# Lakonik/SSDNeRF

Hardware: NVIDIA H100
Metric: rays/sec (128^2 render) & DDIM triplanes/sec (higher is better)
Workload: dtype fp16 tensor-core UNet (fp32 accumulate), fp32 renderer

## Files before the change

ssdnerf_b200/csrc/conv_row2.cu:

```cuda
#include "common.cuh"
#include "tc_common.cuh"
#include "conv_row_epilogue.cuh"
#include "../../include/ssdnerf_b200.h"
#include <cuda_fp16.h>

namespace ssdnerf {
using namespace tc;

constexpr int kRwThreads = 384;
constexpr int kRwRowSlot = 17 * 1024;
constexpr int kRwBSlot = kRwN * 128;
constexpr int kRwRows = 6, kRwBStages = 6;
constexpr size_t kRwSmem = (size_t)kRwRows * kRwRowSlot + (size_t)kRwBStages * kRwBSlot + 1024  + 256  +
                           256  + 512 ;

struct ConvRowParams {
    uint32_t B, H;
    const __half* x1; uint32_t C1;
    const __half* x2; uint32_t C2;
    long long xs1[3], xs2[3];
    const float* bias;
    const __half* residual;
    __half* out;
    float* qstats;
};

__global__ void __launch_bounds__(kRwThreads, 1)
k_conv_row2(const __grid_constant__ CUtensorMap mapB, const ConvRowParams p) {
    extern __shared__ uint8_t smem_raw[];
    uint8_t* smem = reinterpret_cast<uint8_t*>(((uintptr_t)smem_raw + 1023) & ~(uintptr_t)1023);
    uint8_t* sR = smem;
    uint8_t* sB = smem + kRwRows * kRwRowSlot;
    uint64_t* fullR = reinterpret_cast<uint64_t*>(sB + kRwBStages * kRwBSlot);
    uint64_t* emptyR = fullR + kRwRows;
    uint64_t* fullB = emptyR + kRwRows;
    uint64_t* emptyB = fullB + kRwBStages;
    float* qacc = reinterpret_cast<float*>(reinterpret_cast<uint8_t*>(fullR) + 256);
    float* sbias = qacc + 64;

    const int warp = threadIdx.x >> 5, lane = threadIdx.x & 31, wg = warp >> 2;
    const uint32_t tiles_per_img = p.H / 2, total_tiles = p.B * tiles_per_img;
    const uint32_t kc1 = p.C1 / 64, KC = (p.C1 + p.C2) / 64;
    const uint32_t tile0 = blockIdx.x, tstep = gridDim.x;
    const uint32_t my_tiles = tile0 < total_tiles ? (total_tiles - tile0 + tstep - 1) / tstep : 0;

    if (threadIdx.x == 0) {
        prefetch_tmap(&mapB);
        for (int i = 0; i < kRwRows; ++i) { mbar_init(&fullR[i], 4); mbar_init(&emptyR[i], 8); }
        for (int i = 0; i < kRwBStages; ++i) { mbar_init(&fullB[i], 1); mbar_init(&emptyB[i], 8); }
        fence_mbar_init();
    }
    for (int i = threadIdx.x; i < 64; i += kRwThreads) qacc[i] = 0.0f;
    for (int i = threadIdx.x; i < kRwN; i += kRwThreads) sbias[i] = p.bias ? __ldg(p.bias + i) : 0.0f;
    __syncthreads();
    pdl_trigger();
    pdl_wait();

    if (wg == 2) {
        setmaxnreg_dec<120>();
        const uint32_t lt = threadIdx.x - 256u;
        const uint32_t c8 = lt & 7u, p0 = lt >> 3;
        uint32_t idx = 0;
        for (uint32_t tile = tile0; tile < total_tiles; tile += tstep) {
            const uint32_t b = tile / tiles_per_img, y0 = (tile - b * tiles_per_img) * 2;
            for (uint32_t j = 0; j < KC; ++j) {
                const bool first = j < kc1;
                const __half* src = first ? p.x1 : p.x2;
                const long long xs0 = first ? p.xs1[0] : p.xs2[0], xs1 = first ? p.xs1[1] : p.xs2[1], xs2 = first ? p.xs1[2] : p.xs2[2];
                const uint32_t cl = (first ? j : j - kc1) * 64u + c8 * 8u;
                for (uint32_t r = 0; r < 4; ++r) {
                    const int y = (int)(y0 + r) - 1;
                    const bool row_ok = y >= 0 && y < (int)p.H;
                    const __half* rowp = src + (long long)b * xs2 + (long long)(row_ok ? y : 0) * xs1 + cl;
                    uint4 v[9];
#pragma unroll
                    for (int n = 0; n < 9; ++n) {
                        const int x = (int)(p0 + 16u * n) - 1;
                        v[n] = (row_ok && (unsigned)x < (unsigned)kRwW) ? __ldg(reinterpret_cast<const uint4*>(rowp + (long long)x * xs0))
                                                                       : make_uint4(0, 0, 0, 0);
                    }
                    const uint32_t slot = idx % kRwRows;
                    mbar_wait(&emptyR[slot], ((idx / kRwRows) & 1u) ^ 1u);
                    const uint32_t dst = smem_u32(sR + slot * kRwRowSlot);
#pragma unroll
                    for (int n = 0; n < 9; ++n) {
                        const uint32_t px = p0 + 16u * n;
                        if (px >= 130u) continue;
                        sts128(dst + px * 128u + ((c8 ^ (px & 7u)) << 4), v[n]);
                    }
                    __syncwarp();
                    if (lane == 0) mbar_arrive(&fullR[slot]);
                    ++idx;
                }
            }
        }
    } else {
        setmaxnreg_inc<192>();
        const uint32_t a = (uint32_t)wg, wq = (uint32_t)warp & 3u, cq = (uint32_t)lane & 3u;
        const uint32_t steps_per_tile = KC * 9u, total_steps = my_tiles * steps_per_tile;
        auto issue_w = [&](uint32_t L) {
            const uint32_t s = L % kRwBStages;
            if (L >= (uint32_t)kRwBStages) mbar_wait(&emptyB[s], ((L / kRwBStages) - 1u) & 1u);
            mbar_expect_tx(&fullB[s], (uint32_t)kRwBSlot);
            const uint32_t rem = L % steps_per_tile;
            tma_load_4d(sB + s * kRwBSlot, &mapB, &fullB[s], (int)((rem / 9u) * 64u), 0, (int)(rem % 9u), 0);
        };
        if (threadIdx.x == 0)
            for (uint32_t L = 0; L < total_steps && L < (uint32_t)kRwBStages; ++L) issue_w(L);
        auto release_row = [&](uint32_t ring) { if (lane == 0) mbar_arrive(&emptyR[ring % kRwRows]); };
        uint32_t m = 0, ridx = 0;
        const uint32_t lrow = wq * 16u + ((uint32_t)lane & 15u);
        const uint32_t lk = (uint32_t)lane >> 4;
        for (uint32_t tile = tile0; tile < total_tiles; tile += tstep) {
            const uint32_t b = tile / tiles_per_img, y0 = (tile - b * tiles_per_img) * 2;
            float acc0[64], acc1[64];
#pragma unroll
            for (int i = 0; i < 64; ++i) { acc0[i] = 0.0f; acc1[i] = 0.0f; }
            for (uint32_t j = 0; j < KC; ++j) {
                const uint32_t unused = ridx + (a == 0 ? 3u : 0u);
                if (a == 1) { mbar_wait(&fullR[unused % kRwRows], (unused / kRwRows) & 1u); release_row(unused); }
                for (uint32_t ky = 0; ky < 3; ++ky) {
                    const uint32_t ring = ridx + ky + a;
                    mbar_wait(&fullR[ring % kRwRows], (ring / kRwRows) & 1u);
                    const uint32_t rowS = smem_u32(sR + (ring % kRwRows) * kRwRowSlot);
                    for (uint32_t kx = 0; kx < 3; ++kx) {
                        const uint32_t sb = m % kRwBStages;
                        uint32_t af[2][4][4];
#pragma unroll
                        for (uint32_t h = 0; h < 2; ++h) {
                            const uint32_t px = 64u * h + lrow + kx;
#pragma unroll
                            for (uint32_t k = 0; k < 4; ++k) ldmatrix_x4(rowS + px * 128u + (((2u * k + lk) ^ (px & 7u)) << 4), af[h][k]);
                        }
                        if (kx == 2) release_row(ring);
                        mbar_wait(&fullB[sb], (m / kRwBStages) & 1u);
                        const uint64_t b_desc = make_desc_sw128(smem_u32(sB + sb * kRwBSlot));
                        wgmma_fence();
                        fence_regs(acc0); fence_regs(acc1);
#pragma unroll
                        for (uint32_t k = 0; k < 4; ++k) {
                            wgmma_rs_n128(acc0, af[0][k], b_desc + 2 * k, 1u);
                            wgmma_rs_n128(acc1, af[1][k], b_desc + 2 * k, 1u);
                        }
                        wgmma_commit();
                        wgmma_wait<0>();
                        fence_regs(acc0); fence_regs(acc1);
                        if (lane == 0) mbar_arrive(&emptyB[sb]);
                        if (threadIdx.x == 0 && m >= 1 && m - 1 + kRwBStages < total_steps) issue_w(m - 1 + kRwBStages);
                        ++m;
                    }
                }
                if (a == 0) { mbar_wait(&fullR[unused % kRwRows], (unused / kRwRows) & 1u); release_row(unused); }
                ridx += 4;
            }
            const size_t pix0 = ((size_t)b * p.H + y0 + a) * kRwW;
#pragma unroll
            for (int i = 0; i < 16; ++i) {
                const uint32_t ch = 8u * i + 2u * cq;
                const float b0 = sbias[ch], b1 = sbias[ch + 1];
                float su = 0.0f, sq = 0.0f;
#pragma unroll
                for (int h = 0; h < 2; ++h) {
#pragma unroll
                    for (int hh = 0; hh < 2; ++hh) {
                        const size_t o = (pix0 + 64u * h + wq * 16u + ((uint32_t)lane >> 2) + 8u * hh) * kRwN + ch;
                        float v0 = (h ? acc1 : acc0)[4 * i + 2 * hh] + b0, v1 = (h ? acc1 : acc0)[4 * i + 2 * hh + 1] + b1;
                        if (p.residual) { const float2 r = __half22float2(*reinterpret_cast<const __half2*>(p.residual + o)); v0 += r.x; v1 += r.y; }
                        *reinterpret_cast<__half2*>(p.out + o) = __floats2half2_rn(v0, v1);
                        su += v0 + v1; sq = fmaf(v0, v0, fmaf(v1, v1, sq));
                    }
                }
                if (p.qstats) {
                    frag_quad_reduce(su, sq);
                    if ((lane & ~2) == 0) { float* qa = qacc + (2 * i + (lane >> 1)) * 2; atomicAdd(qa, su); atomicAdd(qa + 1, sq); }
                }
            }
            if (p.qstats) {
                asm volatile("bar.sync 1, 256;" ::: "memory");
                if (threadIdx.x < 64) {
                    const float val = qacc[threadIdx.x];
                    if (val != 0.0f) atomicAdd(p.qstats + (size_t)b * 64 + threadIdx.x, val);
                    qacc[threadIdx.x] = 0.0f;
                }
                asm volatile("bar.sync 1, 256;" ::: "memory");
            }
        }
    }
    __syncthreads();
}

int make_map_4d_box(CUtensorMap* m, const void* base, uint64_t K, uint64_t e1, uint64_t e2, uint64_t e3, uint64_t s1, uint64_t s2, uint64_t s3,
                    uint32_t x1, uint32_t x2, uint32_t x3);

static int launch_row2(const CUtensorMap& mB, const ConvRowParams& p, int sms, cudaStream_t stream) {
    static DeviceOnce attr;
    if (attr.first()) {
        SSDNERF_CUDA_OK(cudaFuncSetAttribute(k_conv_row2, cudaFuncAttributeMaxDynamicSharedMemorySize, (int)kRwSmem));
    }
    const uint32_t total = p.B * (p.H / 2);
    SSDNERF_CUDA_OK(launch_pdl(k_conv_row2, dim3(total < (uint32_t)sms ? total : (uint32_t)sms), dim3(kRwThreads), kRwSmem, stream, mB, p));
    SSDNERF_LAUNCH_OK();
    return 0;
}

int conv_row2_launch(const ssdnerf_gemm_args* a, int sms, cudaStream_t stream) {
    if (((uintptr_t)a->a1 & 15u) || ((a->a1_strides[0] | a->a1_strides[1] | a->a1_strides[2]) & 15u) ||
        (a->a2 && (((uintptr_t)a->a2 & 15u) || ((a->a2_strides[0] | a->a2_strides[1] | a->a2_strides[2]) & 15u))) ||
        ((uintptr_t)a->out & 3u) || ((uintptr_t)a->residual & 3u))
        return set_error_msg(SSDNERF_ERR_ARG, "gemm: row-pair convolution needs 16-byte aligned inputs and strides, 4-byte aligned output / residual");
    ConvRowParams p{};
    p.B = a->d3; p.H = a->d2;
    p.x1 = (const __half*)a->a1; p.C1 = a->k1;
    p.x2 = (const __half*)a->a2; p.C2 = a->a2 ? a->k2 : 0;
    for (int i = 0; i < 3; ++i) { p.xs1[i] = (long long)(a->a1_strides[i] / 2); p.xs2[i] = a->a2 ? (long long)(a->a2_strides[i] / 2) : 0; }
    p.bias = a->bias_n; p.residual = (const __half*)a->residual; p.out = (__half*)a->out; p.qstats = a->qstats;
    const uint64_t ktot = (uint64_t)a->k1 + (a->a2 ? a->k2 : 0);
    CUtensorMap mB;
    if (int e = make_map_4d_box(&mB, a->b, ktot, a->n_rows_b ? a->n_rows_b : a->n, a->bx2 ? a->bx2 : 1, a->bx3 ? a->bx3 : 1, a->b_strides[0],
                                a->b_strides[1], a->b_strides[2], kRwN, 1, 1)) return e;
    return launch_row2(mB, p, sms, stream);
}

}
```

ssdnerf_b200/csrc/tc_common.cuh:

```cuda
#pragma once
#include <cuda.h>
#include <cuda_runtime.h>
#include <stdint.h>

namespace ssdnerf {
namespace tc {

__device__ __forceinline__ uint32_t smem_u32(const void* p) { return (uint32_t)__cvta_generic_to_shared(p); }

__device__ __forceinline__ void sts128(uint32_t addr, const uint4& v) {
    asm volatile("st.shared.v4.b32 [%0], {%1, %2, %3, %4};" ::"r"(addr), "r"(v.x), "r"(v.y), "r"(v.z), "r"(v.w) : "memory");
}

__device__ __forceinline__ void mbar_init(uint64_t* bar, uint32_t count) {
    asm volatile("mbarrier.init.shared::cta.b64 [%0], %1;" ::"r"(smem_u32(bar)), "r"(count));
}
__device__ __forceinline__ void fence_mbar_init() { asm volatile("fence.mbarrier_init.release.cluster;" ::: "memory"); }
__device__ __forceinline__ void mbar_arrive(uint64_t* bar) {
    asm volatile("mbarrier.arrive.shared::cta.b64 _, [%0];" ::"r"(smem_u32(bar)) : "memory");
}
__device__ __forceinline__ void mbar_wait(uint64_t* bar, uint32_t parity) {
    uint32_t spins = 0, ok = 0;
    while (!ok) {
        asm volatile(
            "{\n\t.reg .pred p;\n\t"
            "mbarrier.try_wait.parity.acquire.cluster.shared::cta.b64 p, [%1], %2;\n\t"
            "selp.b32 %0, 1, 0, p;\n\t}"
            : "=r"(ok) : "r"(smem_u32(bar)), "r"(parity) : "memory");
        if (!ok && ++spins > 200000000u) { asm volatile("trap;"); }
    }
}
__device__ __forceinline__ void mbar_expect_tx(uint64_t* bar, uint32_t bytes) {
    asm volatile("mbarrier.arrive.expect_tx.shared::cta.b64 _, [%0], %1;" ::"r"(smem_u32(bar)), "r"(bytes) : "memory");
}

__device__ __forceinline__ void prefetch_tmap(const CUtensorMap* m) {
    asm volatile("prefetch.tensormap [%0];" ::"l"(reinterpret_cast<uint64_t>(m)) : "memory");
}
__device__ __forceinline__ void tma_load_4d(void* dst, const CUtensorMap* m, uint64_t* bar, int c0, int c1, int c2, int c3) {
    asm volatile(
        "cp.async.bulk.tensor.4d.shared::cluster.global.mbarrier::complete_tx::bytes [%0], [%1, {%3, %4, %5, %6}], [%2];"
        ::"r"(smem_u32(dst)), "l"(reinterpret_cast<uint64_t>(m)), "r"(smem_u32(bar)), "r"(c0), "r"(c1), "r"(c2), "r"(c3)
        : "memory");
}
__device__ __forceinline__ void fence_proxy_async_smem() { asm volatile("fence.proxy.async.shared::cta;" ::: "memory"); }

template <int N> __device__ __forceinline__ void setmaxnreg_inc() { asm volatile("setmaxnreg.inc.sync.aligned.u32 %0;" ::"n"(N)); }
template <int N> __device__ __forceinline__ void setmaxnreg_dec() { asm volatile("setmaxnreg.dec.sync.aligned.u32 %0;" ::"n"(N)); }

__device__ __forceinline__ uint64_t make_desc_sw128(uint32_t smem_addr) {
    uint64_t d = 0;
    d |= (uint64_t)((smem_addr >> 4) & 0x3FFFu);
    d |= (uint64_t)1 << 16;
    d |= (uint64_t)(1024u >> 4) << 32;
    d |= (uint64_t)1 << 62;
    return d;
}
__device__ __forceinline__ void wgmma_fence() { asm volatile("wgmma.fence.sync.aligned;" ::: "memory"); }
__device__ __forceinline__ void wgmma_commit() { asm volatile("wgmma.commit_group.sync.aligned;" ::: "memory"); }
template <int N> __device__ __forceinline__ void wgmma_wait() { asm volatile("wgmma.wait_group.sync.aligned %0;" ::"n"(N) : "memory"); }
template <int R> __device__ __forceinline__ void fence_regs(float (&d)[R]) {
#pragma unroll
    for (int i = 0; i < R; ++i) asm volatile("" : "+f"(d[i])::"memory");
}

__device__ __forceinline__ void ldmatrix_x4(uint32_t addr, uint32_t (&r)[4]) {
    asm volatile("ldmatrix.sync.aligned.m8n8.x4.shared.b16 {%0, %1, %2, %3}, [%4];"
                 : "=r"(r[0]), "=r"(r[1]), "=r"(r[2]), "=r"(r[3]) : "r"(addr) : "memory");
}

__device__ __forceinline__ void wgmma_ss_n64(float (&d)[32], uint64_t a_desc, uint64_t b_desc, uint32_t accumulate) {
    asm volatile(
        "{\n\t.reg .pred p;\n\t"
        "setp.ne.b32 p, %34, 0;\n\t"
        "wgmma.mma_async.sync.aligned.m64n64k16.f32.f16.f16 "
        "{%0, %1, %2, %3, %4, %5, %6, %7, %8, %9, %10, %11, %12, %13, %14, %15, %16, %17, %18, %19, %20, %21, %22, %23, %24, %25, %26, %27, %28, %29, %30, %31}, %32, %33, p, 1, 1, 0, 0;\n\t}"
        : "+f"(d[0]), "+f"(d[1]), "+f"(d[2]), "+f"(d[3]), "+f"(d[4]), "+f"(d[5]), "+f"(d[6]), "+f"(d[7]), "+f"(d[8]), "+f"(d[9]), "+f"(d[10]), "+f"(d[11]), "+f"(d[12]), "+f"(d[13]), "+f"(d[14]), "+f"(d[15]), "+f"(d[16]), "+f"(d[17]), "+f"(d[18]), "+f"(d[19]), "+f"(d[20]), "+f"(d[21]), "+f"(d[22]), "+f"(d[23]), "+f"(d[24]), "+f"(d[25]), "+f"(d[26]), "+f"(d[27]), "+f"(d[28]), "+f"(d[29]), "+f"(d[30]), "+f"(d[31])
        : "l"(a_desc), "l"(b_desc), "r"(accumulate));
}
__device__ __forceinline__ void wgmma_ss_n128(float (&d)[64], uint64_t a_desc, uint64_t b_desc, uint32_t accumulate) {
    asm volatile(
        "{\n\t.reg .pred p;\n\t"
        "setp.ne.b32 p, %66, 0;\n\t"
        "wgmma.mma_async.sync.aligned.m64n128k16.f32.f16.f16 "
        "{%0, %1, %2, %3, %4, %5, %6, %7, %8, %9, %10, %11, %12, %13, %14, %15, %16, %17, %18, %19, %20, %21, %22, %23, %24, %25, %26, %27, %28, %29, %30, %31, %32, %33, %34, %35, %36, %37, %38, %39, %40, %41, %42, %43, %44, %45, %46, %47, %48, %49, %50, %51, %52, %53, %54, %55, %56, %57, %58, %59, %60, %61, %62, %63}, %64, %65, p, 1, 1, 0, 0;\n\t}"
        : "+f"(d[0]), "+f"(d[1]), "+f"(d[2]), "+f"(d[3]), "+f"(d[4]), "+f"(d[5]), "+f"(d[6]), "+f"(d[7]), "+f"(d[8]), "+f"(d[9]), "+f"(d[10]), "+f"(d[11]), "+f"(d[12]), "+f"(d[13]), "+f"(d[14]), "+f"(d[15]), "+f"(d[16]), "+f"(d[17]), "+f"(d[18]), "+f"(d[19]), "+f"(d[20]), "+f"(d[21]), "+f"(d[22]), "+f"(d[23]), "+f"(d[24]), "+f"(d[25]), "+f"(d[26]), "+f"(d[27]), "+f"(d[28]), "+f"(d[29]), "+f"(d[30]), "+f"(d[31]), "+f"(d[32]), "+f"(d[33]), "+f"(d[34]), "+f"(d[35]), "+f"(d[36]), "+f"(d[37]), "+f"(d[38]), "+f"(d[39]), "+f"(d[40]), "+f"(d[41]), "+f"(d[42]), "+f"(d[43]), "+f"(d[44]), "+f"(d[45]), "+f"(d[46]), "+f"(d[47]), "+f"(d[48]), "+f"(d[49]), "+f"(d[50]), "+f"(d[51]), "+f"(d[52]), "+f"(d[53]), "+f"(d[54]), "+f"(d[55]), "+f"(d[56]), "+f"(d[57]), "+f"(d[58]), "+f"(d[59]), "+f"(d[60]), "+f"(d[61]), "+f"(d[62]), "+f"(d[63])
        : "l"(a_desc), "l"(b_desc), "r"(accumulate));
}
__device__ __forceinline__ void wgmma_rs_n128(float (&d)[64], const uint32_t (&a)[4], uint64_t b_desc, uint32_t accumulate) {
    asm volatile(
        "{\n\t.reg .pred p;\n\t"
        "setp.ne.b32 p, %69, 0;\n\t"
        "wgmma.mma_async.sync.aligned.m64n128k16.f32.f16.f16 "
        "{%0, %1, %2, %3, %4, %5, %6, %7, %8, %9, %10, %11, %12, %13, %14, %15, %16, %17, %18, %19, %20, %21, %22, %23, %24, %25, %26, %27, %28, %29, %30, %31, %32, %33, %34, %35, %36, %37, %38, %39, %40, %41, %42, %43, %44, %45, %46, %47, %48, %49, %50, %51, %52, %53, %54, %55, %56, %57, %58, %59, %60, %61, %62, %63}, {%64, %65, %66, %67}, %68, p, 1, 1, 0;\n\t}"
        : "+f"(d[0]), "+f"(d[1]), "+f"(d[2]), "+f"(d[3]), "+f"(d[4]), "+f"(d[5]), "+f"(d[6]), "+f"(d[7]), "+f"(d[8]), "+f"(d[9]), "+f"(d[10]), "+f"(d[11]), "+f"(d[12]), "+f"(d[13]), "+f"(d[14]), "+f"(d[15]), "+f"(d[16]), "+f"(d[17]), "+f"(d[18]), "+f"(d[19]), "+f"(d[20]), "+f"(d[21]), "+f"(d[22]), "+f"(d[23]), "+f"(d[24]), "+f"(d[25]), "+f"(d[26]), "+f"(d[27]), "+f"(d[28]), "+f"(d[29]), "+f"(d[30]), "+f"(d[31]), "+f"(d[32]), "+f"(d[33]), "+f"(d[34]), "+f"(d[35]), "+f"(d[36]), "+f"(d[37]), "+f"(d[38]), "+f"(d[39]), "+f"(d[40]), "+f"(d[41]), "+f"(d[42]), "+f"(d[43]), "+f"(d[44]), "+f"(d[45]), "+f"(d[46]), "+f"(d[47]), "+f"(d[48]), "+f"(d[49]), "+f"(d[50]), "+f"(d[51]), "+f"(d[52]), "+f"(d[53]), "+f"(d[54]), "+f"(d[55]), "+f"(d[56]), "+f"(d[57]), "+f"(d[58]), "+f"(d[59]), "+f"(d[60]), "+f"(d[61]), "+f"(d[62]), "+f"(d[63])
        : "r"(a[0]), "r"(a[1]), "r"(a[2]), "r"(a[3]), "l"(b_desc), "r"(accumulate));
}
__device__ __forceinline__ void wgmma_ss_n256(float (&d)[128], uint64_t a_desc, uint64_t b_desc, uint32_t accumulate) {
    asm volatile(
        "{\n\t.reg .pred p;\n\t"
        "setp.ne.b32 p, %130, 0;\n\t"
        "wgmma.mma_async.sync.aligned.m64n256k16.f32.f16.f16 "
        "{%0, %1, %2, %3, %4, %5, %6, %7, %8, %9, %10, %11, %12, %13, %14, %15, %16, %17, %18, %19, %20, %21, %22, %23, %24, %25, %26, %27, %28, %29, %30, %31, %32, %33, %34, %35, %36, %37, %38, %39, %40, %41, %42, %43, %44, %45, %46, %47, %48, %49, %50, %51, %52, %53, %54, %55, %56, %57, %58, %59, %60, %61, %62, %63, %64, %65, %66, %67, %68, %69, %70, %71, %72, %73, %74, %75, %76, %77, %78, %79, %80, %81, %82, %83, %84, %85, %86, %87, %88, %89, %90, %91, %92, %93, %94, %95, %96, %97, %98, %99, %100, %101, %102, %103, %104, %105, %106, %107, %108, %109, %110, %111, %112, %113, %114, %115, %116, %117, %118, %119, %120, %121, %122, %123, %124, %125, %126, %127}, %128, %129, p, 1, 1, 0, 0;\n\t}"
        : "+f"(d[0]), "+f"(d[1]), "+f"(d[2]), "+f"(d[3]), "+f"(d[4]), "+f"(d[5]), "+f"(d[6]), "+f"(d[7]), "+f"(d[8]), "+f"(d[9]), "+f"(d[10]), "+f"(d[11]), "+f"(d[12]), "+f"(d[13]), "+f"(d[14]), "+f"(d[15]), "+f"(d[16]), "+f"(d[17]), "+f"(d[18]), "+f"(d[19]), "+f"(d[20]), "+f"(d[21]), "+f"(d[22]), "+f"(d[23]), "+f"(d[24]), "+f"(d[25]), "+f"(d[26]), "+f"(d[27]), "+f"(d[28]), "+f"(d[29]), "+f"(d[30]), "+f"(d[31]), "+f"(d[32]), "+f"(d[33]), "+f"(d[34]), "+f"(d[35]), "+f"(d[36]), "+f"(d[37]), "+f"(d[38]), "+f"(d[39]), "+f"(d[40]), "+f"(d[41]), "+f"(d[42]), "+f"(d[43]), "+f"(d[44]), "+f"(d[45]), "+f"(d[46]), "+f"(d[47]), "+f"(d[48]), "+f"(d[49]), "+f"(d[50]), "+f"(d[51]), "+f"(d[52]), "+f"(d[53]), "+f"(d[54]), "+f"(d[55]), "+f"(d[56]), "+f"(d[57]), "+f"(d[58]), "+f"(d[59]), "+f"(d[60]), "+f"(d[61]), "+f"(d[62]), "+f"(d[63]), "+f"(d[64]), "+f"(d[65]), "+f"(d[66]), "+f"(d[67]), "+f"(d[68]), "+f"(d[69]), "+f"(d[70]), "+f"(d[71]), "+f"(d[72]), "+f"(d[73]), "+f"(d[74]), "+f"(d[75]), "+f"(d[76]), "+f"(d[77]), "+f"(d[78]), "+f"(d[79]), "+f"(d[80]), "+f"(d[81]), "+f"(d[82]), "+f"(d[83]), "+f"(d[84]), "+f"(d[85]), "+f"(d[86]), "+f"(d[87]), "+f"(d[88]), "+f"(d[89]), "+f"(d[90]), "+f"(d[91]), "+f"(d[92]), "+f"(d[93]), "+f"(d[94]), "+f"(d[95]), "+f"(d[96]), "+f"(d[97]), "+f"(d[98]), "+f"(d[99]), "+f"(d[100]), "+f"(d[101]), "+f"(d[102]), "+f"(d[103]), "+f"(d[104]), "+f"(d[105]), "+f"(d[106]), "+f"(d[107]), "+f"(d[108]), "+f"(d[109]), "+f"(d[110]), "+f"(d[111]), "+f"(d[112]), "+f"(d[113]), "+f"(d[114]), "+f"(d[115]), "+f"(d[116]), "+f"(d[117]), "+f"(d[118]), "+f"(d[119]), "+f"(d[120]), "+f"(d[121]), "+f"(d[122]), "+f"(d[123]), "+f"(d[124]), "+f"(d[125]), "+f"(d[126]), "+f"(d[127])
        : "l"(a_desc), "l"(b_desc), "r"(accumulate));
}

__device__ __forceinline__ void wgmma_ss_n16(float (&d)[8], uint64_t a_desc, uint64_t b_desc, uint32_t accumulate) {
    asm volatile(
        "{\n\t.reg .pred p;\n\t"
        "setp.ne.b32 p, %10, 0;\n\t"
        "wgmma.mma_async.sync.aligned.m64n16k16.f32.f16.f16 "
        "{%0, %1, %2, %3, %4, %5, %6, %7}, %8, %9, p, 1, 1, 0, 0;\n\t}"
        : "+f"(d[0]), "+f"(d[1]), "+f"(d[2]), "+f"(d[3]), "+f"(d[4]), "+f"(d[5]), "+f"(d[6]), "+f"(d[7])
        : "l"(a_desc), "l"(b_desc), "r"(accumulate));
}
__device__ __forceinline__ void wgmma_ss_n40(float (&d)[20], uint64_t a_desc, uint64_t b_desc, uint32_t accumulate) {
    asm volatile(
        "{\n\t.reg .pred p;\n\t"
        "setp.ne.b32 p, %22, 0;\n\t"
        "wgmma.mma_async.sync.aligned.m64n40k16.f32.f16.f16 "
        "{%0, %1, %2, %3, %4, %5, %6, %7, %8, %9, %10, %11, %12, %13, %14, %15, %16, %17, %18, %19}, %20, %21, p, 1, 1, 0, 0;\n\t}"
        : "+f"(d[0]), "+f"(d[1]), "+f"(d[2]), "+f"(d[3]), "+f"(d[4]), "+f"(d[5]), "+f"(d[6]), "+f"(d[7]), "+f"(d[8]), "+f"(d[9]), "+f"(d[10]), "+f"(d[11]), "+f"(d[12]), "+f"(d[13]), "+f"(d[14]), "+f"(d[15]), "+f"(d[16]), "+f"(d[17]), "+f"(d[18]), "+f"(d[19])
        : "l"(a_desc), "l"(b_desc), "r"(accumulate));
}
__device__ __forceinline__ void wgmma_ss_n48(float (&d)[24], uint64_t a_desc, uint64_t b_desc, uint32_t accumulate) {
    asm volatile(
        "{\n\t.reg .pred p;\n\t"
        "setp.ne.b32 p, %26, 0;\n\t"
        "wgmma.mma_async.sync.aligned.m64n48k16.f32.f16.f16 "
        "{%0, %1, %2, %3, %4, %5, %6, %7, %8, %9, %10, %11, %12, %13, %14, %15, %16, %17, %18, %19, %20, %21, %22, %23}, %24, %25, p, 1, 1, 0, 0;\n\t}"
        : "+f"(d[0]), "+f"(d[1]), "+f"(d[2]), "+f"(d[3]), "+f"(d[4]), "+f"(d[5]), "+f"(d[6]), "+f"(d[7]), "+f"(d[8]), "+f"(d[9]), "+f"(d[10]), "+f"(d[11]), "+f"(d[12]), "+f"(d[13]), "+f"(d[14]), "+f"(d[15]), "+f"(d[16]), "+f"(d[17]), "+f"(d[18]), "+f"(d[19]), "+f"(d[20]), "+f"(d[21]), "+f"(d[22]), "+f"(d[23])
        : "l"(a_desc), "l"(b_desc), "r"(accumulate));
}
__device__ __forceinline__ void wgmma_ss_n80(float (&d)[40], uint64_t a_desc, uint64_t b_desc, uint32_t accumulate) {
    asm volatile(
        "{\n\t.reg .pred p;\n\t"
        "setp.ne.b32 p, %42, 0;\n\t"
        "wgmma.mma_async.sync.aligned.m64n80k16.f32.f16.f16 "
        "{%0, %1, %2, %3, %4, %5, %6, %7, %8, %9, %10, %11, %12, %13, %14, %15, %16, %17, %18, %19, %20, %21, %22, %23, %24, %25, %26, %27, %28, %29, %30, %31, %32, %33, %34, %35, %36, %37, %38, %39}, %40, %41, p, 1, 1, 0, 0;\n\t}"
        : "+f"(d[0]), "+f"(d[1]), "+f"(d[2]), "+f"(d[3]), "+f"(d[4]), "+f"(d[5]), "+f"(d[6]), "+f"(d[7]), "+f"(d[8]), "+f"(d[9]), "+f"(d[10]), "+f"(d[11]), "+f"(d[12]), "+f"(d[13]), "+f"(d[14]), "+f"(d[15]), "+f"(d[16]), "+f"(d[17]), "+f"(d[18]), "+f"(d[19]), "+f"(d[20]), "+f"(d[21]), "+f"(d[22]), "+f"(d[23]), "+f"(d[24]), "+f"(d[25]), "+f"(d[26]), "+f"(d[27]), "+f"(d[28]), "+f"(d[29]), "+f"(d[30]), "+f"(d[31]), "+f"(d[32]), "+f"(d[33]), "+f"(d[34]), "+f"(d[35]), "+f"(d[36]), "+f"(d[37]), "+f"(d[38]), "+f"(d[39])
        : "l"(a_desc), "l"(b_desc), "r"(accumulate));
}
__device__ __forceinline__ void wgmma_ss_n160(float (&d)[80], uint64_t a_desc, uint64_t b_desc, uint32_t accumulate) {
    asm volatile(
        "{\n\t.reg .pred p;\n\t"
        "setp.ne.b32 p, %82, 0;\n\t"
        "wgmma.mma_async.sync.aligned.m64n160k16.f32.f16.f16 "
        "{%0, %1, %2, %3, %4, %5, %6, %7, %8, %9, %10, %11, %12, %13, %14, %15, %16, %17, %18, %19, %20, %21, %22, %23, %24, %25, %26, %27, %28, %29, %30, %31, %32, %33, %34, %35, %36, %37, %38, %39, %40, %41, %42, %43, %44, %45, %46, %47, %48, %49, %50, %51, %52, %53, %54, %55, %56, %57, %58, %59, %60, %61, %62, %63, %64, %65, %66, %67, %68, %69, %70, %71, %72, %73, %74, %75, %76, %77, %78, %79}, %80, %81, p, 1, 1, 0, 0;\n\t}"
        : "+f"(d[0]), "+f"(d[1]), "+f"(d[2]), "+f"(d[3]), "+f"(d[4]), "+f"(d[5]), "+f"(d[6]), "+f"(d[7]), "+f"(d[8]), "+f"(d[9]), "+f"(d[10]), "+f"(d[11]), "+f"(d[12]), "+f"(d[13]), "+f"(d[14]), "+f"(d[15]), "+f"(d[16]), "+f"(d[17]), "+f"(d[18]), "+f"(d[19]), "+f"(d[20]), "+f"(d[21]), "+f"(d[22]), "+f"(d[23]), "+f"(d[24]), "+f"(d[25]), "+f"(d[26]), "+f"(d[27]), "+f"(d[28]), "+f"(d[29]), "+f"(d[30]), "+f"(d[31]), "+f"(d[32]), "+f"(d[33]), "+f"(d[34]), "+f"(d[35]), "+f"(d[36]), "+f"(d[37]), "+f"(d[38]), "+f"(d[39]), "+f"(d[40]), "+f"(d[41]), "+f"(d[42]), "+f"(d[43]), "+f"(d[44]), "+f"(d[45]), "+f"(d[46]), "+f"(d[47]), "+f"(d[48]), "+f"(d[49]), "+f"(d[50]), "+f"(d[51]), "+f"(d[52]), "+f"(d[53]), "+f"(d[54]), "+f"(d[55]), "+f"(d[56]), "+f"(d[57]), "+f"(d[58]), "+f"(d[59]), "+f"(d[60]), "+f"(d[61]), "+f"(d[62]), "+f"(d[63]), "+f"(d[64]), "+f"(d[65]), "+f"(d[66]), "+f"(d[67]), "+f"(d[68]), "+f"(d[69]), "+f"(d[70]), "+f"(d[71]), "+f"(d[72]), "+f"(d[73]), "+f"(d[74]), "+f"(d[75]), "+f"(d[76]), "+f"(d[77]), "+f"(d[78]), "+f"(d[79])
        : "l"(a_desc), "l"(b_desc), "r"(accumulate));
}

}
}
```

Before: 97.87 million.

## Switch row conv to SS wgmma with one-deep async pipelining and batched residual loads

Replaces the ldmatrix-fed register-A wgmma with shared-memory descriptors for A, which removes the per-step ldmatrix traffic and register pressure. It keeps one wgmma group in flight (wait<1>) and defers releasing B stages and rows until the next step, so the tensor cores no longer stall on each step's completion. Because the producer's generic stores are now read by the async proxy, it adds a proxy fence. The epilogue also batches the residual loads ahead of use. In exchange, weight prefetch is issued one stage later, and the 130-pixel row layout must line up with the SW128 descriptor stride.

```diff
diff --git a/ssdnerf_b200/csrc/conv_row2.cu b/ssdnerf_b200/csrc/conv_row2.cu
--- a/ssdnerf_b200/csrc/conv_row2.cu
+++ b/ssdnerf_b200/csrc/conv_row2.cu
@@ -88,6 +88,7 @@
                         if (px >= 130u) continue;
                         sts128(dst + px * 128u + ((c8 ^ (px & 7u)) << 4), v[n]);
                     }
+                    fence_proxy_async_smem();
                     __syncwarp();
                     if (lane == 0) mbar_arrive(&fullR[slot]);
                     ++idx;
@@ -108,9 +109,14 @@
         if (threadIdx.x == 0)
             for (uint32_t L = 0; L < total_steps && L < (uint32_t)kRwBStages; ++L) issue_w(L);
         auto release_row = [&](uint32_t ring) { if (lane == 0) mbar_arrive(&emptyR[ring % kRwRows]); };
+        constexpr uint32_t kNone = 0xFFFFFFFFu;
+        uint32_t pend_b = kNone, pend_row = kNone;
+        auto retire = [&]() {
+            if (pend_b != kNone && lane == 0) mbar_arrive(&emptyB[pend_b]);
+            if (pend_row != kNone) release_row(pend_row);
+            pend_b = kNone; pend_row = kNone;
+        };
         uint32_t m = 0, ridx = 0;
-        const uint32_t lrow = wq * 16u + ((uint32_t)lane & 15u);
-        const uint32_t lk = (uint32_t)lane >> 4;
         for (uint32_t tile = tile0; tile < total_tiles; tile += tstep) {
             const uint32_t b = tile / tiles_per_img, y0 = (tile - b * tiles_per_img) * 2;
             float acc0[64], acc1[64];
@@ -125,54 +131,69 @@
                     const uint32_t rowS = smem_u32(sR + (ring % kRwRows) * kRwRowSlot);
                     for (uint32_t kx = 0; kx < 3; ++kx) {
                         const uint32_t sb = m % kRwBStages;
-                        uint32_t af[2][4][4];
-#pragma unroll
-                        for (uint32_t h = 0; h < 2; ++h) {
-                            const uint32_t px = 64u * h + lrow + kx;
-#pragma unroll
-                            for (uint32_t k = 0; k < 4; ++k) ldmatrix_x4(rowS + px * 128u + (((2u * k + lk) ^ (px & 7u)) << 4), af[h][k]);
-                        }
-                        if (kx == 2) release_row(ring);
+                        const uint64_t a_desc0 = make_desc_sw128(rowS + kx * 128u), a_desc1 = make_desc_sw128(rowS + (64u + kx) * 128u);
                         mbar_wait(&fullB[sb], (m / kRwBStages) & 1u);
                         const uint64_t b_desc = make_desc_sw128(smem_u32(sB + sb * kRwBSlot));
                         wgmma_fence();
                         fence_regs(acc0); fence_regs(acc1);
 #pragma unroll
                         for (uint32_t k = 0; k < 4; ++k) {
-                            wgmma_rs_n128(acc0, af[0][k], b_desc + 2 * k, 1u);
-                            wgmma_rs_n128(acc1, af[1][k], b_desc + 2 * k, 1u);
+                            wgmma_ss_n128(acc0, a_desc0 + 2 * k, b_desc + 2 * k, 1u);
+                            wgmma_ss_n128(acc1, a_desc1 + 2 * k, b_desc + 2 * k, 1u);
                         }
                         wgmma_commit();
-                        wgmma_wait<0>();
                         fence_regs(acc0); fence_regs(acc1);
-                        if (lane == 0) mbar_arrive(&emptyB[sb]);
-                        if (threadIdx.x == 0 && m >= 1 && m - 1 + kRwBStages < total_steps) issue_w(m - 1 + kRwBStages);
+                        wgmma_wait<1>();
+                        retire();
+                        pend_b = sb;
+                        pend_row = kx == 2 ? ring : kNone;
+                        if (threadIdx.x == 0 && m >= 2 && m - 2 + kRwBStages < total_steps) issue_w(m - 2 + kRwBStages);
                         ++m;
                     }
                 }
                 if (a == 0) { mbar_wait(&fullR[unused % kRwRows], (unused / kRwRows) & 1u); release_row(unused); }
                 ridx += 4;
             }
+            wgmma_wait<0>();
+            fence_regs(acc0); fence_regs(acc1);
+            retire();
             const size_t pix0 = ((size_t)b * p.H + y0 + a) * kRwW;
-#pragma unroll
-            for (int i = 0; i < 16; ++i) {
-                const uint32_t ch = 8u * i + 2u * cq;
-                const float b0 = sbias[ch], b1 = sbias[ch + 1];
-                float su = 0.0f, sq = 0.0f;
-#pragma unroll
-                for (int h = 0; h < 2; ++h) {
-#pragma unroll
-                    for (int hh = 0; hh < 2; ++hh) {
-                        const size_t o = (pix0 + 64u * h + wq * 16u + ((uint32_t)lane >> 2) + 8u * hh) * kRwN + ch;
-                        float v0 = (h ? acc1 : acc0)[4 * i + 2 * hh] + b0, v1 = (h ? acc1 : acc0)[4 * i + 2 * hh + 1] + b1;
-                        if (p.residual) { const float2 r = __half22float2(*reinterpret_cast<const __half2*>(p.residual + o)); v0 += r.x; v1 += r.y; }
-                        *reinterpret_cast<__half2*>(p.out + o) = __floats2half2_rn(v0, v1);
-                        su += v0 + v1; sq = fmaf(v0, v0, fmaf(v1, v1, sq));
-                    }
-                }
-                if (p.qstats) {
-                    frag_quad_reduce(su, sq);
-                    if ((lane & ~2) == 0) { float* qa = qacc + (2 * i + (lane >> 1)) * 2; atomicAdd(qa, su); atomicAdd(qa + 1, sq); }
+            auto out_off = [&](int i, int h, int hh) {
+                return (pix0 + 64u * h + wq * 16u + ((uint32_t)lane >> 2) + 8u * hh) * kRwN + 8u * i + 2u * cq;
+            };
+            constexpr int kRwResBatch = 8;
+#pragma unroll
+            for (int i0 = 0; i0 < 16; i0 += kRwResBatch) {
+                __half2 res[kRwResBatch][2][2];
+                if (p.residual) {
+#pragma unroll
+                    for (int ii = 0; ii < kRwResBatch; ++ii)
+#pragma unroll
+                        for (int h = 0; h < 2; ++h)
+#pragma unroll
+                            for (int hh = 0; hh < 2; ++hh) res[ii][h][hh] = *reinterpret_cast<const __half2*>(p.residual + out_off(i0 + ii, h, hh));
+                }
+#pragma unroll
+                for (int ii = 0; ii < kRwResBatch; ++ii) {
+                    const int i = i0 + ii;
+                    const uint32_t ch = 8u * i + 2u * cq;
+                    const float b0 = sbias[ch], b1 = sbias[ch + 1];
+                    float su = 0.0f, sq = 0.0f;
+#pragma unroll
+                    for (int h = 0; h < 2; ++h) {
+#pragma unroll
+                        for (int hh = 0; hh < 2; ++hh) {
+                            const size_t o = out_off(i, h, hh);
+                            float v0 = (h ? acc1 : acc0)[4 * i + 2 * hh] + b0, v1 = (h ? acc1 : acc0)[4 * i + 2 * hh + 1] + b1;
+                            if (p.residual) { const float2 r = __half22float2(res[ii][h][hh]); v0 += r.x; v1 += r.y; }
+                            *reinterpret_cast<__half2*>(p.out + o) = __floats2half2_rn(v0, v1);
+                            su += v0 + v1; sq = fmaf(v0, v0, fmaf(v1, v1, sq));
+                        }
+                    }
+                    if (p.qstats) {
+                        frag_quad_reduce(su, sq);
+                        if ((lane & ~2) == 0) { float* qa = qacc + (2 * i + (lane >> 1)) * 2; atomicAdd(qa, su); atomicAdd(qa + 1, sq); }
+                    }
                 }
             }
             if (p.qstats) {
diff --git a/ssdnerf_b200/csrc/tc_common.cuh b/ssdnerf_b200/csrc/tc_common.cuh
--- a/ssdnerf_b200/csrc/tc_common.cuh
+++ b/ssdnerf_b200/csrc/tc_common.cuh
@@ -64,11 +64,6 @@
     for (int i = 0; i < R; ++i) asm volatile("" : "+f"(d[i])::"memory");
 }
 
-__device__ __forceinline__ void ldmatrix_x4(uint32_t addr, uint32_t (&r)[4]) {
-    asm volatile("ldmatrix.sync.aligned.m8n8.x4.shared.b16 {%0, %1, %2, %3}, [%4];"
-                 : "=r"(r[0]), "=r"(r[1]), "=r"(r[2]), "=r"(r[3]) : "r"(addr) : "memory");
-}
-
 __device__ __forceinline__ void wgmma_ss_n64(float (&d)[32], uint64_t a_desc, uint64_t b_desc, uint32_t accumulate) {
     asm volatile(
         "{\n\t.reg .pred p;\n\t"
@@ -86,15 +81,6 @@
         "{%0, %1, %2, %3, %4, %5, %6, %7, %8, %9, %10, %11, %12, %13, %14, %15, %16, %17, %18, %19, %20, %21, %22, %23, %24, %25, %26, %27, %28, %29, %30, %31, %32, %33, %34, %35, %36, %37, %38, %39, %40, %41, %42, %43, %44, %45, %46, %47, %48, %49, %50, %51, %52, %53, %54, %55, %56, %57, %58, %59, %60, %61, %62, %63}, %64, %65, p, 1, 1, 0, 0;\n\t}"
         : "+f"(d[0]), "+f"(d[1]), "+f"(d[2]), "+f"(d[3]), "+f"(d[4]), "+f"(d[5]), "+f"(d[6]), "+f"(d[7]), "+f"(d[8]), "+f"(d[9]), "+f"(d[10]), "+f"(d[11]), "+f"(d[12]), "+f"(d[13]), "+f"(d[14]), "+f"(d[15]), "+f"(d[16]), "+f"(d[17]), "+f"(d[18]), "+f"(d[19]), "+f"(d[20]), "+f"(d[21]), "+f"(d[22]), "+f"(d[23]), "+f"(d[24]), "+f"(d[25]), "+f"(d[26]), "+f"(d[27]), "+f"(d[28]), "+f"(d[29]), "+f"(d[30]), "+f"(d[31]), "+f"(d[32]), "+f"(d[33]), "+f"(d[34]), "+f"(d[35]), "+f"(d[36]), "+f"(d[37]), "+f"(d[38]), "+f"(d[39]), "+f"(d[40]), "+f"(d[41]), "+f"(d[42]), "+f"(d[43]), "+f"(d[44]), "+f"(d[45]), "+f"(d[46]), "+f"(d[47]), "+f"(d[48]), "+f"(d[49]), "+f"(d[50]), "+f"(d[51]), "+f"(d[52]), "+f"(d[53]), "+f"(d[54]), "+f"(d[55]), "+f"(d[56]), "+f"(d[57]), "+f"(d[58]), "+f"(d[59]), "+f"(d[60]), "+f"(d[61]), "+f"(d[62]), "+f"(d[63])
         : "l"(a_desc), "l"(b_desc), "r"(accumulate));
-}
-__device__ __forceinline__ void wgmma_rs_n128(float (&d)[64], const uint32_t (&a)[4], uint64_t b_desc, uint32_t accumulate) {
-    asm volatile(
-        "{\n\t.reg .pred p;\n\t"
-        "setp.ne.b32 p, %69, 0;\n\t"
-        "wgmma.mma_async.sync.aligned.m64n128k16.f32.f16.f16 "
-        "{%0, %1, %2, %3, %4, %5, %6, %7, %8, %9, %10, %11, %12, %13, %14, %15, %16, %17, %18, %19, %20, %21, %22, %23, %24, %25, %26, %27, %28, %29, %30, %31, %32, %33, %34, %35, %36, %37, %38, %39, %40, %41, %42, %43, %44, %45, %46, %47, %48, %49, %50, %51, %52, %53, %54, %55, %56, %57, %58, %59, %60, %61, %62, %63}, {%64, %65, %66, %67}, %68, p, 1, 1, 0;\n\t}"
-        : "+f"(d[0]), "+f"(d[1]), "+f"(d[2]), "+f"(d[3]), "+f"(d[4]), "+f"(d[5]), "+f"(d[6]), "+f"(d[7]), "+f"(d[8]), "+f"(d[9]), "+f"(d[10]), "+f"(d[11]), "+f"(d[12]), "+f"(d[13]), "+f"(d[14]), "+f"(d[15]), "+f"(d[16]), "+f"(d[17]), "+f"(d[18]), "+f"(d[19]), "+f"(d[20]), "+f"(d[21]), "+f"(d[22]), "+f"(d[23]), "+f"(d[24]), "+f"(d[25]), "+f"(d[26]), "+f"(d[27]), "+f"(d[28]), "+f"(d[29]), "+f"(d[30]), "+f"(d[31]), "+f"(d[32]), "+f"(d[33]), "+f"(d[34]), "+f"(d[35]), "+f"(d[36]), "+f"(d[37]), "+f"(d[38]), "+f"(d[39]), "+f"(d[40]), "+f"(d[41]), "+f"(d[42]), "+f"(d[43]), "+f"(d[44]), "+f"(d[45]), "+f"(d[46]), "+f"(d[47]), "+f"(d[48]), "+f"(d[49]), "+f"(d[50]), "+f"(d[51]), "+f"(d[52]), "+f"(d[53]), "+f"(d[54]), "+f"(d[55]), "+f"(d[56]), "+f"(d[57]), "+f"(d[58]), "+f"(d[59]), "+f"(d[60]), "+f"(d[61]), "+f"(d[62]), "+f"(d[63])
-        : "r"(a[0]), "r"(a[1]), "r"(a[2]), "r"(a[3]), "l"(b_desc), "r"(accumulate));
 }
 __device__ __forceinline__ void wgmma_ss_n256(float (&d)[128], uint64_t a_desc, uint64_t b_desc, uint32_t accumulate) {
     asm volatile(
```

Result: no change. 97.67 million, median of 6 (-0.2%).
